# Rinoahu/SwiftOrtho

Hardware: AMD Instinct MI355X
Metric: M query-aa/s scanned all-vs-all (higher is better)
Workload: dtype u8/int16/int32 (5-bit packed residues, packed 16-bit score-only DP, int32 traced DP); 1 GPU; BASELINE config 3: 100000 synthetic proteins x 300 aa self-search, seed 11111011111, aa9, -M 120000000, -c 50000 (2 chunks), -e 1e-5, -v 500; query_aa=30007201, rows=1618760

## Files before the change

### include/sohit.h

```cpp
#ifndef SOHIT_H
#define SOHIT_H

#include <stdint.h>

#ifdef __cplusplus
extern "C" {
#endif

#define SOHIT_ABI_VERSION 3

typedef struct so_ctx so_ctx;

typedef struct so_params {
    const char *seeds;
    const char *alphabet;
    int64_t nc;
    int64_t chunk;
    int64_t step;
    int64_t max_hits;
    int64_t thr;
    double expect;
    double max_miss;
    int32_t filter;
    int32_t profile;
// ... 35 lines not shown
    int64_t bounds_bytes;
    int64_t align_launches;
    double align_ms;
    double index_ms, seed_ms, group_ms, phase2_ms, total_ms;
    int64_t count_launches;
    double count_ms;
    int64_t hits_bucketed;
    int64_t align_wide;
    int64_t cells_wide;
    int64_t seed_passes;
    int64_t ungap_steps;
    int64_t groups_single;
    int64_t groups_chain;
    int64_t bgroup_launches;
    double bgroup_ms;
} so_counters;

so_ctx *so_create(int device, const so_params *params);
void so_destroy(so_ctx *ctx);
const char *so_last_error(const so_ctx *ctx);
int so_abi_version(void);
int so_set_option(so_ctx *ctx, const char *name, const char *value);

int so_load_ref(so_ctx *ctx, const char *fasta_path, int64_t r_lo, int64_t r_hi);
int so_load_ref_mem(so_ctx *ctx, const char *fasta_bytes, int64_t nbytes, int64_t r_lo, int64_t r_hi);
int so_build_index(so_ctx *ctx);
int so_drop_index(so_ctx *ctx);
int so_load_index(so_ctx *ctx, const char *prefix);

int so_load_queries(so_ctx *ctx, const char *fasta_path);
// ... 83 lines not shown
```

### swiftortho_amd/_lib.py

```python
import ctypes as C
import os

HERE = os.path.dirname(os.path.abspath(__file__))
LIBPATH = os.path.join(HERE, "libsohit.so")


class SoParams(C.Structure):
    _fields_ = [("seeds", C.c_char_p), ("alphabet", C.c_char_p), ("nc", C.c_int64), ("chunk", C.c_int64), ("step", C.c_int64),
                ("max_hits", C.c_int64), ("thr", C.c_int64), ("expect", C.c_double), ("max_miss", C.c_double),
                ("filter", C.c_int32), ("profile", C.c_int32)]


class SoHit(C.Structure):
    _fields_ = [("qidx", C.c_int64), ("sidx", C.c_int64), ("identity", C.c_double), ("evalue", C.c_double), ("aln", C.c_int32),
                ("mis", C.c_int32), ("gap", C.c_int32), ("qst", C.c_int32), ("qed", C.c_int32), ("sst", C.c_int32),
                ("sed", C.c_int32), ("bit", C.c_int32), ("qlen", C.c_int32), ("slen", C.c_int32), ("matches", C.c_int32),
                ("ungapped", C.c_int32)]


class SoCounters(C.Structure):
    _fields_ = [(n, C.c_int64) for n in ("n_queries", "query_aa", "ref_seqs", "ref_aa", "n_chunks", "seed_windows", "seed_hits",
                                         "groups", "candidates", "alignments", "cells", "rows", "index_entries")] + \
               [("lookup_launches", C.c_int64), ("lookup_ms", C.c_double), ("lookup_bytes", C.c_int64),
                ("bounds_launches", C.c_int64), ("bounds_ms", C.c_double), ("bounds_bytes", C.c_int64),
                ("align_launches", C.c_int64), ("align_ms", C.c_double),
                ("index_ms", C.c_double), ("seed_ms", C.c_double), ("group_ms", C.c_double), ("phase2_ms", C.c_double),
                ("total_ms", C.c_double), ("count_launches", C.c_int64), ("count_ms", C.c_double),
                ("hits_bucketed", C.c_int64), ("align_wide", C.c_int64), ("cells_wide", C.c_int64), ("seed_passes", C.c_int64),
                ("ungap_steps", C.c_int64), ("groups_single", C.c_int64), ("groups_chain", C.c_int64),
                ("bgroup_launches", C.c_int64), ("bgroup_ms", C.c_double)]

    def as_dict(self):
        return {n: getattr(self, n) for n, _ in self._fields_}


EXPORTS = ["so_abi_version", "so_set_option", "so_create", "so_destroy", "so_last_error", "so_load_ref", "so_load_ref_mem", "so_build_index", "so_drop_index", "so_load_index",
           "so_load_queries", "so_load_queries_mem", "so_num_queries", "so_num_refs", "so_query_len", "so_search_loaded",
           "so_search", "so_free_hits", "so_search_loaded_aln", "so_free_aln", "so_write_sc", "so_format_hit", "so_get_counters", "so_reset_counters", "so_timing_report",
           "so_chunk_threshold", "so_chunk_entries", "so_chunk_download", "so_masked_query", "so_query_candidates", "so_align_pairs", "so_align_pairs_aln", "so_set_profile",
           "so_bucket_count", "so_ref_len", "so_search_device", "so_device_hits_copy", "so_query_work", "so_mcl", "so_mcl_free",
           "so_mcl_last_error", "so_tsv_lines", "so_tsv_scan", "so_tsv_codes", "so_format_pairs", "so_py_repr", "so_fmt_rows",
           "so_search_loaded_cigar", "so_free_cigar", "so_format_cigar", "so_write_sc_cigar", "so_align_pairs_cigar",
           "so_apc", "so_apc_free", "so_apc_last_error"]


# ... 118 lines not shown
```

### swiftortho_amd/build.py

```python
import concurrent.futures
import os
import subprocess
import sys

HERE = os.path.dirname(os.path.abspath(__file__))
CSRC = os.path.join(HERE, "csrc")
OBJ = os.path.join(HERE, "_build")
LIB = os.path.join(HERE, "libsohit.so")
INCLUDE = os.path.join(os.path.dirname(HERE), "include")
HIPCC = os.environ.get("HIPCC", "/opt/rocm/bin/hipcc")
ARCH = "gfx950"

SOURCES = ["k_util.hip", "k_sort.hip", "k_sortseg.hip", "k_prep.hip", "k_index.hip", "k_ixsort.hip", "k_seed.hip", "k_group.hip", "k_ungap1.hip", "k_ungapq.hip", "k_bucket.hip", "k_align.hip", "k_align16.hip", "k_alignl.hip", "k_phase2.hip", "mcl.hip", "apc.hip",
           "tsv.hip", "host_load.hip", "host_index.hip", "host_seed.hip", "host_phase2.hip", "host_search.hip", "host_abi.hip"]
FLAGS = ["-O3", "-std=c++17", "-fPIC", "--offload-arch=" + ARCH, "-ffp-contract=off", "-Wall", "-Wno-unused-function",
         "-Wno-unused-result", "-I", CSRC, "-I", INCLUDE] + os.environ.get("SOHIT_CXXFLAGS", "").split()


def _deps_mtime():
    m = 0.0
    for d in (CSRC, INCLUDE):
        for f in os.listdir(d):
            if f.endswith((".h", ".hpp")):
                m = max(m, os.path.getmtime(os.path.join(d, f)))
    return m


def _compile(src, force):
# ... 33 lines not shown
```

### swiftortho_amd/csrc/host.h

```cpp
#pragma once
#include "common.h"
#include "kernels.h"
#include "seedhash.h"
#include "../../include/sohit.h"

#include <algorithm>
#include <array>
#include <atomic>
#include <chrono>
#include <cmath>
#include <cstring>
#include <functional>
#include <map>
#include <malloc.h>
#include <memory>
#include <mutex>
#include <thread>
#include <unordered_map>
#include <sys/stat.h>

inline double wall() { return std::chrono::duration<double>(std::chrono::steady_clock::now().time_since_epoch()).count(); }

extern double (*volatile p_pow)(double, double);
extern double (*volatile p_log)(double);
// ... 116 lines not shown
    };
    std::vector<std::unique_ptr<RangeTab>> rtabs;
};


#define EMIT_PARTS_MAX 8
enum SmallSlot : int {
    SM_STASH0 = 0, SM_STASH1 = 1,
    SM_SEED_TOTAL = 2,
    SM_ANY_RANK = 3,
    SM_PART_ROW = 4,
    SM_WIDE_ROUND = 12,
    SM_LANE_CTR = 13,
    SM_FLAG = 14,
    SM_WIDE_PART = 16,
    SM_WORDS = 32
};
static_assert(SM_PART_ROW > SM_ANY_RANK && SM_PART_ROW + EMIT_PARTS_MAX <= SM_WIDE_ROUND, "d_small: emission rows");
static_assert(SM_WIDE_PART > SM_FLAG && SM_WIDE_PART + EMIT_PARTS_MAX <= SM_WORDS, "d_small: wide counts per range");

struct so_ctx {
    int device = 0;
    u32 ncu = 256;
    Tune tune;
    hipStream_t st = nullptr;
    std::string seeds, alphabet;
    i64 nc = 0, chunk = 50000, step = 1, v = 500, thr = -1;
    double expect = 1e-3, max_miss = 1e-3;
    bool filter = true, profile = false;
    SeedCfg cfg;
    std::vector<std::array<int, 256>> codes;
    std::string err;
    DevBuf<u8> d_smap, d_hmap;
    DevBuf<signed char> d_b62c;
// ... 163 lines not shown
    DevBuf<u32> cand_q, cand_rec;
    std::vector<u32> chunk_base;
    DevBuf<u32> ccnt;
    DevBuf<unsigned long long> qcells;
    DevBuf<u32> tpos, spcnt, spoff, sidx, spec_trace, sel_a, sel_b;
    DevBuf<u64> gx;
    DevBuf<u32> gL, gR;
    DevBuf<u32> segfirst, st_state, rcnt, tcnt, roff, ridx, ridx2, ntile, roffc, rk_slot, order_tmp;
    DevBuf<u32> cqoff, prior, qtot, qcoff, fin_rec, perm, ntask, toff, sel, nout, ooff;
    DevBuf<AlnTask> tasks;
    DevBuf<AlnRes> ares;
    DevBuf<int> bits, outrec;
    DevBuf<u32> trace;
    DevBuf<u32> tr_units, tr_ofs;
    DevBuf<u32> tl_sorted, al_sorted;
    AlnChain aln;
};

#define QCLASSES 5
static_assert(QCLASSES <= QCLASSES_MAX, "Batch::cls_start");
inline u8 query_class(u32 len) { return len < 512 ? 0 : len < 1024 ? 1 : len < 2048 ? 2 : len < 4096 ? 3 : 4; }

struct StageClock {
    so_ctx* c;
    double t = 0;
    explicit StageClock(so_ctx* c_) : c(c_) {
        if (c->profile) {
            (void)hipStreamSynchronize(c->st);
            t = wall();
        }
// ... 270 lines not shown
```

### swiftortho_amd/csrc/host_phase2.hip

```cpp
#include "host.h"


void aln_decode(const u32* w, int AL, const u8* qp, const u8* sp, char* sq, char* ss) {
    for (int f = 0; f < AL; ++f) {
        const int cc = AL - 1 - f;
        const u32 code = (w[cc >> 4] >> ((cc & 15) << 1)) & 3u;
        sq[f] = code != 2 ? (char)*qp++ : '-';
        ss[f] = code != 3 ? (char)*sp++ : '-';
    }
}

void emit_join(so_ctx* c, HitBuf& out) {
    if (!c->emit.active) return;
    c->emit.th.join();
    c->emit.active = false;
    if (c->emit.err) {
        std::exception_ptr e = c->emit.err;
        c->emit.err = nullptr;
        std::rethrow_exception(e);
    }
    if (c->emit.dropped.load()) {
        const double expect = c->expect;
        if (c->emit.cig) {
            CigarBuf& g = out.cig;
// ... 69 lines not shown
template <class F>
static std::vector<size_t> aln_word_offsets(size_t n, F aln_at, size_t words, const char* who) {
    std::vector<size_t> w(n + 1, 0);
    for (size_t i = 0; i < n; ++i) w[i + 1] = w[i] + (size_t)(std::max(0, (int)aln_at(i)) + 15) / 16;
    if (w[n] != words) throw SoError(std::string(who) + ": column words do not add up");
    return w;
}

struct P2 {
    P2(so_ctx* c, const Batch& b) : sc(c), nq(b.nq) {}
    const double t0 = wall();
    StageClock sc;
    u32 nq, Ntot = 0, NT = 0, nspec = 0, NO = 0;
    AlnSeqs seqs{};
    bool align_sort = false, pk_on = false, pk_mixed = false, lane_on = false, traced_pk = false, aln_on = false, cig_on = false;
    u32 stride = 0, slab = 0, TU = 0;
    size_t var_budget_words = 0, aln_words = 0, cig_ops = 0;
    int parts = 1; u32 qstep = 0;
    std::array<u32, EMIT_PARTS_MAX + 1> part_row{};
    std::vector<u32> h_ooff;
};

static bool gather_candidates(so_ctx* c, Batch& b, P2& p) {
    const int nchunks = (int)c->chunks.size();
    const u32 nq = p.nq;
    const u32 Ntot = p.Ntot = b.chunk_base.empty() ? 0u : b.chunk_base.back();
    b.qtot.ensure((size_t)nq + 4), b.qcoff.ensure((size_t)nq + 4), b.prior.ensure((size_t)nq + 4), b.cqoff.ensure((size_t)nq + 4);
    HIP_CHECK(hipMemsetAsync(b.qtot.p, 0, ((size_t)nq + 4) * sizeof(u32), c->st));
    for (int ci = 0; ci < nchunks; ++ci) launch_add_u32(b.qtot.p, b.ccnt.p + (size_t)ci * nq, nq, c->st);
    c->d_scan_tmp.ensure(scan_u32_temp_elems((size_t)nq + 1) + 8);
// ... 11 lines not shown
        launch_add_u32(b.prior.p, cc, nq, c->st);
    }
    p.sc.lap("phase2.gather");
    if (tune().keep_cands) {
        std::vector<u32> qcoff((size_t)nq + 1), rec(4 * (size_t)Ntot + 4);
        HIP_CHECK(hipMemcpyAsync(qcoff.data(), b.qcoff.p, ((size_t)nq + 1) * sizeof(u32), hipMemcpyDeviceToHost, c->st));
        if (Ntot) HIP_CHECK(hipMemcpyAsync(rec.data(), b.fin_rec.p, 4 * (size_t)Ntot * sizeof(u32), hipMemcpyDeviceToHost, c->st));
        HIP_CHECK(hipStreamSynchronize(c->st));
        for (u32 q = 0; q < nq; ++q) {
            auto& dst = c->last_cands[(size_t)(b.q_lo - c->last_q_lo) + b.qid[q]];
            dst.assign(rec.begin() + 4 * (size_t)qcoff[q], rec.begin() + 4 * (size_t)qcoff[q + 1]);
        }
    }
    return Ntot != 0;
}

static void make_tasks(so_ctx* c, Batch& b, P2& p) {
    const u32 nq = p.nq, Ntot = p.Ntot;
    const u32 vmax = (u32)std::max<i64>(100, std::max<i64>(c->v + 100, (i64)((double)c->v * 1.1)));
    b.perm.ensure((size_t)Ntot + 4), b.ntask.ensure((size_t)nq + 4), b.ntile.ensure((size_t)nq + 4);
    b.toff.ensure((size_t)nq + 4), b.roffc.ensure((size_t)nq + 4);
    HIP_CHECK(hipMemsetAsync(b.ntask.p, 0, ((size_t)nq + 4) * sizeof(u32), c->st));
    HIP_CHECK(hipMemsetAsync(b.ntile.p, 0, ((size_t)nq + 4) * sizeof(u32), c->st));
    if (c->h_qhits_cap < nq) {
        if (c->h_qhits) (void)hipHostFree(c->h_qhits);
        c->h_qhits_cap = (size_t)nq + 1024;
        HIP_CHECK(hipHostMalloc((void**)&c->h_qhits, c->h_qhits_cap * sizeof(unsigned long long), hipHostMallocDefault));
    }
    const u32* qt = reinterpret_cast<const u32*>(c->h_qhits);
    HIP_CHECK(hipMemcpyAsync(c->h_qhits, b.qtot.p, (size_t)nq * sizeof(u32), hipMemcpyDeviceToHost, c->st));
// ... 35 lines not shown
    p.pk_on = tune().align_pk && align_pk_supported(c->st);
    p.pk_mixed = p.pk_on && (int)std::min(maxwin_q, maxwin_s) > align_pk_max_len();
    p.seqs = AlnSeqs{aln_side(b.dev), aln_side(c->ref), c->d_b62c.p};
    p.lane_on = p.pk_on && tune().align_lane && b.maxqlen < LONG_SEQ && c->ref.maxlen < LONG_SEQ;
    p.traced_pk = p.pk_on;
    p.stride = align_trace_stride((int)std::min<u32>(std::max(maxwin_q, maxwin_s), std::min(maxwin_q, maxwin_s) + 16) + 1);
    const long long trace_var_max = tune().trace_var_max;
    const size_t budget_words = trace_var_max >= 0 ? (size_t)trace_var_max : (size_t)1 << 30;
    p.slab = (u32)std::max<size_t>(16, std::min<size_t>(std::max<u32>(NT, 1), budget_words / std::max<u32>(p.stride, 1)));
    p.var_budget_words = trace_var_max >= 0 ? (size_t)trace_var_max : (size_t)1 << 31;
    p.TU = align_trace_unit();
    b.st_state.ensure(5 * (size_t)nq + 8), b.rcnt.ensure((size_t)nq + 4), b.tcnt.ensure((size_t)nq + 4), b.roff.ensure((size_t)nq + 4);
    b.order_tmp.ensure((size_t)nq + 4);
    b.ridx.ensure((size_t)NT + 4);
    HIP_CHECK(hipMemsetAsync(b.st_state.p, 0, (5 * (size_t)nq + 8) * sizeof(u32), c->st));
    p.sc.lap("phase2.mktasks");
}

static void order_by_rows(so_ctx* c, Batch& b, const AlnSeqs& s, const u32* in, u32 n, u32* out, u32* n_wide, unsigned long long* cells) {
    if (!n) return;
    b.tmp64.ensure((size_t)n + 2), b.c_ft2.ensure((size_t)n + 2);
    ensure_sort_tmp(c, sort_pairs_u64_u32_temp_bytes(n, 64));
    launch_task_rows(b.tasks.p, in, n, s, n_wide, cells, b.tmp64.p, c->st);
    sort_pairs_u64_u32(c->d_sort_tmp.p, c->d_sort_tmp.cap, b.tmp64.p, b.c_ft2.p, in, out, n, n_wide ? 14 : 13, c->st);
}

static const u32* round_list(so_ctx* c, Batch& b, const P2& p, const u32* list, u32 n, u32* n_wide) {
    const bool split = n_wide && p.pk_mixed;
    if (n_wide) *n_wide = p.pk_on ? 0u : n;
    if (!split && (!p.align_sort || n < 4096)) return list;
    b.ridx2.ensure((size_t)n + 2);
// ... 13 lines not shown
}

static void align_rounds(so_ctx* c, Batch& b, P2& p) {
    const u32 nq = p.nq, NT = p.NT;
    const AlnSeqs& s = p.seqs;
    u32 aligned_total = 0;
    const bool spec_on = tune().spec >= 0 ? tune().spec != 0 : NT >= (1u << 21);
    const double spec_slack = tune().spec_slack;
    u32 spec_cap = NT;
    if (tune().spec_cap >= 0) spec_cap = (u32)tune().spec_cap;
    if (spec_on) {
        b.tpos.ensure((size_t)NT + 4);
        HIP_CHECK(hipMemsetAsync(b.tpos.p, 0xFF, ((size_t)NT + 4) * sizeof(u32), c->st));
    }
    bool first_round = true;
    for (u32 minr = 8;; minr = minr < 256 ? minr * 2 : minr) {
        u32 NR = 0, RR = 0, NS = 0;
        bool spec_round = spec_on && first_round;
        first_round = false;
        if (spec_round) {
            b.spcnt.ensure((size_t)nq + 4), b.spoff.ensure((size_t)nq + 4), b.sidx.ensure((size_t)NT + 4);
            c->d_small.ensure(SM_WORDS);
            HIP_CHECK(hipMemsetAsync(c->d_small.p + SM_ANY_RANK, 0, sizeof(u32), c->st));
            launch_round_counts_spec(b.ntask.p, b.ntile.p, b.roffc.p, b.rk_slot.p, b.qcoff.p, b.st_state.p, nq, c->max_miss, minr, b.tasks.p, b.toff.p,
                                     b.dev.d_off.p, c->ref.d_off.p, c->d_bittab.p, so_ctx::BITTAB_N, c->ref.N, c->expect * spec_slack, b.rcnt.p, b.tcnt.p, b.spcnt.p,
                                     c->d_small.p + SM_ANY_RANK, c->st);
            stash_u32(c, scan_u32(b.tcnt.p, b.roff.p, (size_t)nq + 1, false, c->d_scan_tmp.p, c->st), SM_STASH0);
            stash_u32(c, scan_u32(b.spcnt.p, b.spoff.p, (size_t)nq + 1, false, c->d_scan_tmp.p, c->st), SM_STASH1);
            u32* v = (u32*)small_host(c);
            HIP_CHECK(hipMemcpyAsync(v, c->d_small.p, (SM_ANY_RANK + 1) * sizeof(u32), hipMemcpyDeviceToHost, c->st));
            HIP_CHECK(hipStreamSynchronize(c->st));
            NR = v[SM_STASH0], NS = v[SM_STASH1], RR = v[SM_ANY_RANK];
            if (NS > spec_cap) spec_round = false;
        }
        if (!spec_round) {
            NS = 0;
            launch_round_counts(b.ntask.p, b.ntile.p, b.roffc.p, b.rk_slot.p, b.qcoff.p, b.st_state.p, nq, c->max_miss, minr, b.rcnt.p,
                                b.tcnt.p, c->st);
            const u32* dNR = scan_u32(b.tcnt.p, b.roff.p, (size_t)nq + 1, false, c->d_scan_tmp.p, c->st);
            stash_u32(c, dNR, SM_STASH0);
            const u32* dRR = scan_u32(b.rcnt.p, b.order_tmp.p, (size_t)nq + 1, false, c->d_scan_tmp.p, c->st);
            d2h_pair(c, dRR, NR, RR);
        }
        if (RR == 0) break;
        if (spec_round) {
            launch_round_idx_spec(b.tcnt.p, b.spcnt.p, b.roff.p, b.spoff.p, b.toff.p, b.ntask.p, b.ntile.p, b.roffc.p, b.rk_slot.p, b.st_state.p, nq,
                                  b.ridx.p, b.sidx.p, c->st);
            if (NS) {
                u32 nw_s = 0;
                const u32* slist = round_list(c, b, p, b.sidx.p, NS, p.traced_pk ? &nw_s : nullptr);
                if (!p.traced_pk) nw_s = NS;
                const size_t tw = trace_offsets(c, b, p, slist, NS);
                ProfTimer pt(c, &c->cnt.align_ms, &c->cnt.align_launches);
                if (tw <= p.var_budget_words) {
                    b.spec_trace.ensure(tw + 64);
                    launch_align_traced(b.tasks.p, slist, NS, s, b.spec_trace.p, p.TU, b.tr_ofs.p, b.ares.p, b.tpos.p, 0u, c->st, nw_s);
                    p.nspec = NS;
                } else {
                    if (tune().debug) fprintf(stderr, "[sohit] kept traces do not fit: %u tasks scored only\n", NS);
                    launch_align(b.tasks.p, slist, NS, s, b.ares.p, c->st);
                }
                pt.stop();
            }
        } else if (NR) {
            launch_round_idx(b.tcnt.p, b.roff.p, b.toff.p, b.ntask.p, b.ntile.p, b.roffc.p, b.rk_slot.p, b.st_state.p, nq, b.ridx.p, c->st);
        }
        if (NR) {
            u32 n_wide = 0;
            const u32* rlist = round_list(c, b, p, b.ridx.p, NR, &n_wide);
            ProfTimer pt(c, &c->cnt.align_ms, &c->cnt.align_launches);
            const bool wide_aside = n_wide && NR > n_wide;
            hipStream_t wst = wide_aside ? c->st_side : c->st;
            if (wide_aside) {
                HIP_CHECK(hipEventRecord(c->ev_ug_go, c->st));
                HIP_CHECK(hipStreamWaitEvent(c->st_side, c->ev_ug_go, 0));
            }
            if (n_wide) launch_align(b.tasks.p, rlist, n_wide, s, b.ares.p, wst);
            if (wide_aside) HIP_CHECK(hipEventRecord(c->ev_ug_done, c->st_side));
            if (NR > n_wide) {
                if (p.lane_on && (long long)(NR - n_wide) >= tune().align_lane_min) {
                    c->d_small.ensure(SM_WORDS);
                    launch_align_lane(b.tasks.p, rlist + n_wide, NR - n_wide, s, b.ares.p, c->d_small.p + SM_LANE_CTR, c->ncu, c->st);
                } else {
                    launch_align_pk(b.tasks.p, rlist + n_wide, NR - n_wide, s, b.ares.p, c->st);
                }
            }
            if (wide_aside) HIP_CHECK(hipStreamWaitEvent(c->st, c->ev_ug_done, 0));
            pt.stop();
            c->cnt.align_wide += n_wide;
        }
        launch_stop_round_w(b.tasks.p, b.ares.p, b.qcoff.p, b.ntask.p, b.ntile.p, b.roffc.p, b.rk_slot.p, b.toff.p, b.rcnt.p, nq,
                            b.dev.d_off.p, c->ref.d_off.p, c->d_bittab.p, so_ctx::BITTAB_N, c->ref.N, c->expect, c->max_miss, c->v, b.sel.p,
                            b.st_state.p, b.bits.p, b.qcells.p, c->st);
        aligned_total += NR + NS;
    }
    launch_sum_u64(b.qcells.p, nq, b.ucount.p + 1, c->st);
    p.sc.lap("phase2.align_rounds");
    c->cnt.alignments += aligned_total;
}

static void select_rows(so_ctx* c, Batch& b, P2& p) {
    const u32 nq = p.nq;
    b.nout.ensure((size_t)nq + 4), b.ooff.ensure((size_t)nq + 4);
    HIP_CHECK(hipMemsetAsync(b.nout.p, 0xFF, (size_t)nq * sizeof(u32), c->st));
    HIP_CHECK(hipMemsetAsync(b.nout.p + nq, 0, 4 * sizeof(u32), c->st));
    launch_final_select(b.toff.p, nq, c->v, b.sel.p, b.st_state.p, b.bits.p, b.nout.p, c->st);
    const u32* dNO = scan_u32(b.nout.p, b.ooff.p, (size_t)nq + 1, false, c->d_scan_tmp.p, c->st);
    const int emit_parts = std::min<int>(EMIT_PARTS_MAX, std::max(1, (p.nspec && (b.permuted || p.pk_mixed)) ? 2 : (int)tune().emit_parts));
    const u32 emit_min_rows = (u32)std::max(1ll, tune().emit_min_rows);
    const u32 qstep = p.qstep = (nq + emit_parts - 1) / emit_parts;
    c->d_small.ensure(SM_WORDS);
    launch_stride_gather(b.ooff.p, qstep, (nq + qstep - 1) / qstep, c->d_small.p + SM_PART_ROW, c->st);
    stash_u32(c, dNO, SM_STASH0);
// ... 488 lines not shown
```

### swiftortho_amd/csrc/host_search.hip

```cpp
#include "host.h"

HitCache g_hit_cache;
BufCache g_cig_ops_cache, g_cig_off_cache;


void search_loaded(so_ctx* c, i64 q_lo, i64 q_hi, HitBuf& out) {
    if (!c->ref_loaded) throw SoError("so_search: no reference loaded");
    if (!c->qry_loaded) throw SoError("so_search: no queries loaded");
    build_index(c);
    struct EmitGuard {
        so_ctx* c;
        ~EmitGuard() {
            if (c->emit.active) {
                c->emit.th.join();
                c->emit.active = false;
                c->emit.err = nullptr;
            }
        }
    } emit_guard{c};
    const double t0 = wall();
    const i64 N = c->qry.N, D = c->ref.N;
    i64 st = std::min<i64>(std::max<i64>(0, q_lo), N);
    i64 ed = std::min<i64>(q_hi < 0 ? D : q_hi, N);
    if (ed < st) ed = st;
// ... 16 lines not shown
    if (tune().batch <= 0) batch_q = std::min<i64>(batch_q, std::max<i64>(1024, (i64)((double)0xE0000000ull / est_cands)));
    std::function<void(i64, i64)> run_batch = [&](i64 b0, i64 b1) {
        const so_counters keep = c->cnt;
        const size_t keep_rows = out.n, keep_dev_rows = c->d_hits_n;
        try {
            if (!c->batch) c->batch = std::make_shared<Batch>();
            Batch& b = *static_cast<Batch*>(c->batch.get());
            b.chunk_base.clear();
            StageClock scp(c);
            prepare_batch(c, b, b0, b1);
            scp.lap("prepare_batch");
            b.ccnt.ensure((size_t)std::max(1, nchunks) * b.nq + 4);
            HIP_CHECK(hipMemsetAsync(b.ccnt.p, 0, ((size_t)std::max(1, nchunks) * b.nq + 4) * sizeof(u32), c->st));
            for (int ci = 0; ci < nchunks; ++ci) seed_stage(c, b, ci);
            phase2(c, b, out);
            unsigned long long uc[3] = {0, 0, 0};
            HIP_CHECK(hipMemcpyAsync(uc, b.ucount.p, sizeof uc, hipMemcpyDeviceToHost, c->st));
            HIP_CHECK(hipStreamSynchronize(c->st));
            c->cnt.cells += (i64)uc[1];
            c->cnt.cells_wide += (i64)uc[2];
            c->cnt.n_queries += b.nq;
            c->cnt.query_aa += b.h_off[b.nq];
            if (tune().keep_masked) {
                if (c->masked.empty()) c->masked_lo = st;
                if (b.h_res.empty() && b.h_off[b.nq]) {
                    b.h_res.resize(b.h_off[b.nq] + 16);
                    HIP_CHECK(hipMemcpy(b.h_res.data(), b.dev.d_res.p, b.h_off[b.nq], hipMemcpyDeviceToHost));
                }
                const size_t m0 = c->masked.size();
                c->masked.resize(m0 + b.nq);
                for (u32 i = 0; i < b.nq; ++i)
                    c->masked[m0 + b.qid[i]].assign((const char*)b.h_res.data() + b.h_off[i], (size_t)(b.h_off[i + 1] - b.h_off[i]));
            }
        } catch (const SoError& e) {
            const bool oom = dynamic_cast<const DevOom*>(&e) != nullptr;
// ... 54 lines not shown
```

### swiftortho_amd/csrc/kernels.h

```cpp
#pragma once
#include "common.h"

struct HashLut;

size_t scan_u32_temp_elems(size_t n);
size_t effscan_temp_elems(size_t n);
const u32* effscan(const u8* mark, const u32* scnt, size_t n, u32* hoff, u32* cidx, u32* temp, hipStream_t st);
const u32* scan_u32(const u32* in, u32* out, size_t n, bool inclusive, u32* temp, hipStream_t st);
void fill_u32(u32* p, size_t n, u32 v, hipStream_t st);

size_t sort_keys_u64_temp_bytes(size_t n, int bits);
void sort_keys_u64(void* temp, size_t temp_bytes, const u64* in, u64* out, size_t n, int begin_bit, int end_bit, hipStream_t st);
void launch_query_segments(const u32* hoff, const u32* qoff, u32 qa, u32 qb, int AS, u32 H, u32* seg, hipStream_t st);
size_t sort_keys_u64_seg_temp_bytes(size_t n, u32 nseg, int begin_bit, int end_bit);
void sort_keys_u64_seg(void* temp, size_t temp_bytes, const u64* in, u64* out, size_t n, u32 nseg, const u32* seg, int begin_bit,
                       int end_bit, hipStream_t st);
void sort_keys_u64_seg2(void* temp, size_t temp_bytes, const u64* in, u64* out, size_t n, u32 nseg, const u32* seg_begin, const u32* seg_end, int begin_bit,
                        int end_bit, hipStream_t st);
void launch_stride_gather(const u32* src, u32 stride, u32 n, u32* dst, hipStream_t st);
size_t sort_pairs_u64_u32_temp_bytes(size_t n, int bits);
void sort_pairs_u64_u32(void* temp, size_t temp_bytes, const u64* kin, u64* kout, const u32* vin, u32* vout, size_t n, int bits,
                        hipStream_t st);

size_t ixsort_plan_elems(u32 NC);
// ... 188 lines not shown
                           const u32* roffc, const u32* rk_slot, const u32* st_state, u32 nq, u32* ridx, u32* sidx, hipStream_t st);
void launch_trace_flags(const u32* sel_idx, u32 n, const u32* tpos, u32* flags, hipStream_t st);
void launch_trace_split(const u32* sel_idx, u32 n, const u32* flags, const u32* fscan, u32* list_b, u32* list_a, hipStream_t st);
u32 aln_unit_words();
void launch_aln_units(const AlnTask* tasks, const u32* sel_idx, u32 n, const AlnSeqs& s, u32* units , hipStream_t st);
void launch_aln_scatter(const u32* sel_idx, u32 n, const u32* rofs, u32* aofs , hipStream_t st);
void launch_aln_words(const u32* sel_idx, u32 n, const AlnRes* res, u32* words , hipStream_t st);
void launch_aln_compact(const u32* sel_idx, u32 n, const u32* aofs, const u32* acode, const u32* cofs , u32* dst, hipStream_t st);
void launch_cigar_count(const u32* sel_idx, u32 n, const u32* aofs, const u32* acode, const AlnRes* res, u32* runs , hipStream_t st);
void launch_cigar_emit(const u32* sel_idx, u32 n, const u32* aofs, const u32* acode, const AlnRes* res, const u32* op_off , u32* ops, hipStream_t st);
void launch_stop_round_w(const AlnTask* tasks, const AlnRes* res, const u32* qcoff, const u32* ntask, const u32* ntile, const u32* roffc,
                         const u32* rk_slot, const u32* toff, const u32* rcnt, u32 nq, const u32* qoff, const u32* roff, const int* bittab,
                         int bittab_n, i64 D, double expect, double max_miss, i64 v, u32* sel, u32* st_state, int* bits,
                         unsigned long long* qcells , hipStream_t st);
void launch_sum_u64(const unsigned long long* x, u32 n, unsigned long long* total, hipStream_t st);
void launch_task_rows(const AlnTask* tasks, const u32* ridx, u32 n, const AlnSeqs& s, u32* n_wide, unsigned long long* cells_wide ,
                      u64* keys, hipStream_t st);
```

### swiftortho_amd/csrc/tune.h

```cpp
#pragma once
#include <cstdlib>

#define SOHIT_TUNE_TABLE(X)                                                                                                                                     \
                                                                                                                              \
    X(B, ug1, "SOHIT_UG1", 1, "bucketed passes: singleton groups to k_ungap1 (0: everything to k_ungap)")                                                     \
    X(B, ug1_chain, "SOHIT_UG1_CHAIN", 1, "... and the groups of two and more hits to k_ungap2 (0: to k_ungap, which then skips the singletons)")              \
    X(B, count_steps, "SOHIT_UG_COUNT", 0, "counting instances of the extension kernels: so_counters.ungap_steps, groups_single, groups_chain")                \
    X(B, ungapq, "SOHIT_UNGAPQ", 1, "sparse passes of queries up to 512 residues: hits alone on their diagonal by k_ungapq, a wave per query (0: every hit through the sorted keys)")     \
    X(B, ug_w32, "SOHIT_UG_W32", 1, "bucketed passes hand k_ungap the buckets' 32-bit words (0: 64-bit keys; no k_ungap1 then)")                               \
                                                                                                             \
    X(B, bucket, "SOHIT_BUCKET", 1, "bucketed diagonal binning (0: every pass on the sorted path)")                                                            \
    X(I, bucket_min, "SOHIT_BUCKET_MIN", 192, "hits per bucket below which a pass takes the sorted path (0: bucketed whenever possible)")                      \
    X(I, bucket_avg, "SOHIT_BUCKET_AVG", 2560, "average bucket size the band-range width is chosen for")                                                       \
    X(I, count_tab, "SOHIT_COUNT_TAB", 1, "bucketed passes: hits per (tile, range) from the range boundaries of the ordered index buckets when a batch brings a chunk two passes and more (0: always the counting pass over the entries; 2: always both, compared -- tests; 3: always)") \
    X(B, bucket_best, "SOHIT_BUCKET_BEST", 1, "best diagonal per subject by the per-bucket reduction (0: sort of the pass records)")                           \
    X(B, bands, "SOHIT_BANDS", 1, "diagonal bands follow the subjects' lengths (0: one band per subject)")                                                     \
    X(B, lk_wide, "SOHIT_LK_WIDE", 0, "8-byte index addends whatever the field widths")                                                                        \
    X(B, qclass, "SOHIT_QCLASS", 1, "queries of a batch in length-class order (0: file order)")                                                                \
    X(B, pass_merge, "SOHIT_PASS_MERGE", 1, "neighbouring length classes that take the sorted path anyway share one pass")                                     \
    X(B, ksc_lazy, "SOHIT_KSC_LAZY", 1, "k-mer orders computed for the queries that reach their frequency cap, when they do (a query below it keeps every window whatever the order; 0: for every query, with the batch)") \
    X(B, bounds_ahead, "SOHIT_BOUNDS_AHEAD", 1, "the next chunk's bucket bounds (k_bounds) on the side stream beside this chunk's seed stage (0: in front of its own)")     \
    X(I, segsort, "SOHIT_SEGSORT", 1, "sorted path: segmented sort of the keys inside each query (0: device-wide sort)")                                        \
    X(I, write_threads, "SOHIT_WRITE_THREADS", 48, "so_write_sc: formatter threads (at most the host's cores)")                                                                          \
                                                                                                                                 \
    X(I, cand_limit, "SOHIT_CAND_LIMIT", 0, "tests: candidate-store size at which a batch is split (0: 2^32 - 16)")                                            \
                                                                                                                                         \
    X(B, align_pk, "SOHIT_ALIGN_PK", 1, "packed 16-bit score-only aligner where the scores fit")                                                               \
    X(B, align_lane, "SOHIT_ALIGN_LANE", 1, "score-only rounds: one lane per alignment pair (k_align_lane) when no sequence reaches 4096 residues (0: k_align_pk)")            \
    X(I, align_lane_min, "SOHIT_ALIGN_LANE_MIN", 1 << 18, "... for rounds of at least this many packed tasks (below: k_align_pk; tests: 0)")                 \
    X(B, align_sort, "SOHIT_ALIGN_SORT", 1, "launch lists ordered by band rows")                                                                               \
    X(I, trace_wave_rows, "SOHIT_TRACE_WAVE_ROWS", 1024, "traceback: bands of this many rows and more are walked by a wave of their own (0: never)")         \
    X(I, trace_wave_max, "SOHIT_TRACE_WAVE_MAX", 32768, "... among the first this many positions of a launch list")                                            \
    X(I, spec, "SOHIT_SPEC", -1, "speculative traces in the first round: 0 off, 1 on, -1 from 2^21 tasks on")                                                  \
    X(D, spec_slack, "SOHIT_SPEC_SLACK", 1e6, "... the guess tests the ungapped score against expect x this (tests: 1e30 = every first-round task traced, 1e-30 = none)")          \
    X(I, spec_cap, "SOHIT_SPEC_CAP", -1, "tests: most speculative traces kept (-1: all)")                                                                      \
    X(I, trace_var_max, "SOHIT_TRACE_VAR_MAX", -1, "tests: trace words a launch list's own-size traces may take, and the fixed-stride slabs' budget (-1: 2^31 / 2^30)") \
    X(I, emit_parts, "SOHIT_EMIT_PARTS", 4, "... and otherwise")                                                                                               \
    X(I, emit_min_rows, "SOHIT_EMIT_MIN_ROWS", 1 << 18, "rows below which the emission is one part")                                                           \
    X(P, test_oom_phase2, "SOHIT_TEST_OOM_PHASE2", 0, "tests: phase 2 of the first batch fails once with an out-of-memory error")                              \
                                                                                                                                 \
    X(I, batch, "SOHIT_BATCH", 0, "queries per device batch (0: 131072, lowered when the candidate estimate asks)")                                            \
    X(I, max_hits, "SOHIT_MAX_HITS", 0, "seed hits per pass (0: 2^30)")                                                                                        \
    X(I, poison, "SOHIT_POISON", -1, "tests: byte every fresh device allocation is filled with (-1: none)")                                                    \
    X(B, hit_cache, "SOHIT_HIT_CACHE", 1, "one released result array is kept for the next search")                                                             \
    X(P, keep_cands, "SOHIT_KEEP_CANDS", 0, "tests: keep every query's candidate list (so_query_candidates)")                                                  \
    X(P, keep_masked, "SOHIT_KEEP_MASKED", 0, "tests: keep the masked queries (so_masked_query)")                                                              \
    X(I, mcl_scratch, "SOHIT_MCL_SCRATCH", -1, "tests: u32 words of expansion / convergence scratch per range of rows (-1: 2^28)")                             \
                                                                                                                                           \
    X(P, exact_threshold, "SOHIT_EXACT_THRESHOLD", 0, "threshold always by the sequential fp64 replay")                                                        \
    X(I, dir_max, "SOHIT_DIR_MAX", -1, "largest -M served by the bitmap + rank directory (-1: 2^31)")                                                          \
// ... 34 lines not shown
```

Baseline: 670.1 M query-aa/s.

## Reuse mirrored pair scores in all-vs-all score-only alignment rounds

In all-vs-all searches, finds for each score-only alignment task its mirrored task (query and subject swapped, same anchor) through a device hash table. Each round it launches only one task of every mirrored pair and copies the max score and cells to the other, avoiding roughly half of the packed DP work. It adds per-batch identity checks, hash insert/probe kernels, per-round mark/filter/copy kernels and a host sync per round. Eligibility is restricted to full-length, non-symmetric-overhang, non-long tasks so the copied score matches what the kernel would compute.

```diff
diff --git a/include/sohit.h b/include/sohit.h
--- a/include/sohit.h
+++ b/include/sohit.h
@@ -73,6 +73,9 @@
     int64_t groups_chain;
     int64_t bgroup_launches;
     double bgroup_ms;
+    int64_t align_reused;
+    int64_t cells_reused;
+    int64_t align_reused_round;
 } so_counters;
 
 so_ctx *so_create(int device, const so_params *params);
diff --git a/swiftortho_amd/_lib.py b/swiftortho_amd/_lib.py
--- a/swiftortho_amd/_lib.py
+++ b/swiftortho_amd/_lib.py
@@ -28,7 +28,8 @@
                 ("total_ms", C.c_double), ("count_launches", C.c_int64), ("count_ms", C.c_double),
                 ("hits_bucketed", C.c_int64), ("align_wide", C.c_int64), ("cells_wide", C.c_int64), ("seed_passes", C.c_int64),
                 ("ungap_steps", C.c_int64), ("groups_single", C.c_int64), ("groups_chain", C.c_int64),
-                ("bgroup_launches", C.c_int64), ("bgroup_ms", C.c_double)]
+                ("bgroup_launches", C.c_int64), ("bgroup_ms", C.c_double),
+                ("align_reused", C.c_int64), ("cells_reused", C.c_int64), ("align_reused_round", C.c_int64)]
 
     def as_dict(self):
         return {n: getattr(self, n) for n, _ in self._fields_}
diff --git a/swiftortho_amd/build.py b/swiftortho_amd/build.py
--- a/swiftortho_amd/build.py
+++ b/swiftortho_amd/build.py
@@ -11,7 +11,7 @@
 HIPCC = os.environ.get("HIPCC", "/opt/rocm/bin/hipcc")
 ARCH = "gfx950"
 
-SOURCES = ["k_util.hip", "k_sort.hip", "k_sortseg.hip", "k_prep.hip", "k_index.hip", "k_ixsort.hip", "k_seed.hip", "k_group.hip", "k_ungap1.hip", "k_ungapq.hip", "k_bucket.hip", "k_align.hip", "k_align16.hip", "k_alignl.hip", "k_phase2.hip", "mcl.hip", "apc.hip",
+SOURCES = ["k_util.hip", "k_sort.hip", "k_sortseg.hip", "k_prep.hip", "k_index.hip", "k_ixsort.hip", "k_seed.hip", "k_group.hip", "k_ungap1.hip", "k_ungapq.hip", "k_bucket.hip", "k_align.hip", "k_align16.hip", "k_alignl.hip", "k_phase2.hip", "k_pair.hip", "mcl.hip", "apc.hip",
            "tsv.hip", "host_load.hip", "host_index.hip", "host_seed.hip", "host_phase2.hip", "host_search.hip", "host_abi.hip"]
 FLAGS = ["-O3", "-std=c++17", "-fPIC", "--offload-arch=" + ARCH, "-ffp-contract=off", "-Wall", "-Wno-unused-function",
          "-Wno-unused-result", "-I", CSRC, "-I", INCLUDE] + os.environ.get("SOHIT_CXXFLAGS", "").split()
diff --git a/swiftortho_amd/csrc/host.h b/swiftortho_amd/csrc/host.h
--- a/swiftortho_amd/csrc/host.h
+++ b/swiftortho_amd/csrc/host.h
@@ -154,10 +154,11 @@
     SM_LANE_CTR = 13,
     SM_FLAG = 14,
     SM_WIDE_PART = 16,
+    SM_PAIR = 24,
     SM_WORDS = 32
 };
 static_assert(SM_PART_ROW > SM_ANY_RANK && SM_PART_ROW + EMIT_PARTS_MAX <= SM_WIDE_ROUND, "d_small: emission rows");
-static_assert(SM_WIDE_PART > SM_FLAG && SM_WIDE_PART + EMIT_PARTS_MAX <= SM_WORDS, "d_small: wide counts per range");
+static_assert(SM_WIDE_PART > SM_FLAG && SM_WIDE_PART + EMIT_PARTS_MAX <= SM_PAIR && SM_PAIR + 4 <= SM_WORDS, "d_small: wide counts per range, mirrored tasks");
 
 struct so_ctx {
     int device = 0;
@@ -351,6 +352,9 @@
     DevBuf<u32> trace;
     DevBuf<u32> tr_units, tr_ofs;
     DevBuf<u32> tl_sorted, al_sorted;
+    DevBuf<u8> pr_same;
+    DevBuf<u32> pr_partner, pr_state, pr_launch, pr_copy;
+    DevBuf<u64> pr_tab;
     AlnChain aln;
 };
 
diff --git a/swiftortho_amd/csrc/host_phase2.hip b/swiftortho_amd/csrc/host_phase2.hip
--- a/swiftortho_amd/csrc/host_phase2.hip
+++ b/swiftortho_amd/csrc/host_phase2.hip
@@ -107,6 +107,7 @@
     u32 nq, Ntot = 0, NT = 0, nspec = 0, NO = 0;
     AlnSeqs seqs{};
     bool align_sort = false, pk_on = false, pk_mixed = false, lane_on = false, traced_pk = false, aln_on = false, cig_on = false;
+    bool pair_on = false;
     u32 stride = 0, slab = 0, TU = 0;
     size_t var_budget_words = 0, aln_words = 0, cig_ops = 0;
     int parts = 1; u32 qstep = 0;
@@ -148,6 +149,8 @@
     }
     return Ntot != 0;
 }
+
+static bool pair_lookup(so_ctx* c, Batch& b, const P2& p);
 
 static void make_tasks(so_ctx* c, Batch& b, P2& p) {
     const u32 nq = p.nq, Ntot = p.Ntot;
@@ -213,7 +216,28 @@
     b.order_tmp.ensure((size_t)nq + 4);
     b.ridx.ensure((size_t)NT + 4);
     HIP_CHECK(hipMemsetAsync(b.st_state.p, 0, (5 * (size_t)nq + 8) * sizeof(u32), c->st));
+    p.pair_on = p.pk_on && b.maxqlen < LONG_SEQ && c->ref.maxlen < LONG_SEQ && b.q_lo < c->ref.N &&
+                (tune().pair_reuse >= 0 ? tune().pair_reuse != 0 : NT >= (1u << 18)) && pair_lookup(c, b, p);
     p.sc.lap("phase2.mktasks");
+}
+
+static bool pair_lookup(so_ctx* c, Batch& b, const P2& p) {
+    const u32 nq = p.nq, NT = p.NT;
+    c->d_small.ensure(SM_WORDS);
+    b.pr_same.ensure((size_t)nq + 4);
+    HIP_CHECK(hipMemsetAsync(c->d_small.p + SM_PAIR + 3, 0, sizeof(u32), c->st));
+    const u32* qid = b.permuted ? b.d_qid.p : nullptr;
+    launch_pair_same(p.seqs, nq, (u32)b.q_lo, qid, (u32)c->ref.N, b.pr_same.p, c->d_small.p + SM_PAIR + 3, c->st);
+    const u32 n_same = d2h_u32(c, c->d_small.p + SM_PAIR + 3);
+    if (tune().debug) fprintf(stderr, "[sohit] pair reuse: %u of %u queries are their own reference sequences\n", n_same, nq);
+    if (n_same < 2) return false;
+    const size_t entries = pair_table_entries(NT);
+    b.pr_tab.ensure(entries), b.pr_partner.ensure((size_t)NT + 4), b.pr_state.ensure((size_t)NT + 4);
+    b.pr_launch.ensure((size_t)NT + 4), b.pr_copy.ensure((size_t)NT + 4);
+    HIP_CHECK(hipMemsetAsync(b.pr_tab.p, 0xFF, entries * sizeof(u64), c->st));
+    HIP_CHECK(hipMemsetAsync(b.pr_state.p, 0, ((size_t)NT + 4) * sizeof(u32), c->st));
+    launch_pair_lookup(b.tasks.p, NT, p.seqs, b.pr_same.p, (u32)b.q_lo, nq, qid, b.pr_tab.p, b.pr_partner.p, c->st);
+    return true;
 }
 
 static void order_by_rows(so_ctx* c, Batch& b, const AlnSeqs& s, const u32* in, u32 n, u32* out, u32* n_wide, unsigned long long* cells) {
@@ -257,6 +281,8 @@
         HIP_CHECK(hipMemsetAsync(b.tpos.p, 0xFF, ((size_t)NT + 4) * sizeof(u32), c->st));
     }
     bool first_round = true;
+    u32 pair_tag = 0;
+    u32 pair_scored = 0, pair_reused = 0, pair_round = 0;
     for (u32 minr = 8;; minr = minr < 256 ? minr * 2 : minr) {
         u32 NR = 0, RR = 0, NS = 0;
         bool spec_round = spec_on && first_round;
@@ -286,9 +312,30 @@
             d2h_pair(c, dRR, NR, RR);
         }
         if (RR == 0) break;
-        if (spec_round) {
+        if (spec_round)
             launch_round_idx_spec(b.tcnt.p, b.spcnt.p, b.roff.p, b.spoff.p, b.toff.p, b.ntask.p, b.ntile.p, b.roffc.p, b.rk_slot.p, b.st_state.p, nq,
                                   b.ridx.p, b.sidx.p, c->st);
+        else if (NR)
+            launch_round_idx(b.tcnt.p, b.roff.p, b.toff.p, b.ntask.p, b.ntile.p, b.roffc.p, b.rk_slot.p, b.st_state.p, nq, b.ridx.p, c->st);
+        u32 NL = NR;
+        const u32* score_list = b.ridx.p;
+        if (p.pair_on && NR + NS) {
+            ++pair_tag;
+            launch_pair_mark(b.ridx.p, NR, b.sidx.p, NS, pair_tag, b.pr_state.p, c->st);
+            if (NR) {
+                HIP_CHECK(hipMemsetAsync(c->d_small.p + SM_PAIR, 0, 3 * sizeof(u32), c->st));
+                launch_pair_filter(b.ridx.p, NR, pair_tag, b.pr_partner.p, b.pr_state.p, b.pr_launch.p, b.pr_copy.p, c->d_small.p + SM_PAIR, c->st);
+                u32* v = (u32*)small_host(c);
+                HIP_CHECK(hipMemcpyAsync(v, c->d_small.p + SM_PAIR, 3 * sizeof(u32), hipMemcpyDeviceToHost, c->st));
+                HIP_CHECK(hipStreamSynchronize(c->st));
+                NL = v[0];
+                if (NL > NR || v[1] != NR - NL) throw SoError("phase 2: the split of a round's mirrored tasks does not add up");
+                score_list = b.pr_launch.p;
+                pair_scored += NR, pair_reused += NR - NL, pair_round += v[2];
+                if (tune().debug) fprintf(stderr, "[sohit] pair round %u: %u score-only tasks, %u launched, %u copied (%u from this round)\n", pair_tag, NR, NL, NR - NL, v[2]);
+            }
+        }
+        if (spec_round) {
             if (NS) {
                 u32 nw_s = 0;
                 const u32* slist = round_list(c, b, p, b.sidx.p, NS, p.traced_pk ? &nw_s : nullptr);
@@ -305,14 +352,12 @@
                 }
                 pt.stop();
             }
-        } else if (NR) {
-            launch_round_idx(b.tcnt.p, b.roff.p, b.toff.p, b.ntask.p, b.ntile.p, b.roffc.p, b.rk_slot.p, b.st_state.p, nq, b.ridx.p, c->st);
-        }
-        if (NR) {
+        }
+        if (NL) {
             u32 n_wide = 0;
-            const u32* rlist = round_list(c, b, p, b.ridx.p, NR, &n_wide);
+            const u32* rlist = round_list(c, b, p, score_list, NL, &n_wide);
             ProfTimer pt(c, &c->cnt.align_ms, &c->cnt.align_launches);
-            const bool wide_aside = n_wide && NR > n_wide;
+            const bool wide_aside = n_wide && NL > n_wide;
             hipStream_t wst = wide_aside ? c->st_side : c->st;
             if (wide_aside) {
                 HIP_CHECK(hipEventRecord(c->ev_ug_go, c->st));
@@ -320,18 +365,19 @@
             }
             if (n_wide) launch_align(b.tasks.p, rlist, n_wide, s, b.ares.p, wst);
             if (wide_aside) HIP_CHECK(hipEventRecord(c->ev_ug_done, c->st_side));
-            if (NR > n_wide) {
-                if (p.lane_on && (long long)(NR - n_wide) >= tune().align_lane_min) {
+            if (NL > n_wide) {
+                if (p.lane_on && (long long)(NL - n_wide) >= tune().align_lane_min) {
                     c->d_small.ensure(SM_WORDS);
-                    launch_align_lane(b.tasks.p, rlist + n_wide, NR - n_wide, s, b.ares.p, c->d_small.p + SM_LANE_CTR, c->ncu, c->st);
+                    launch_align_lane(b.tasks.p, rlist + n_wide, NL - n_wide, s, b.ares.p, c->d_small.p + SM_LANE_CTR, c->ncu, c->st);
                 } else {
-                    launch_align_pk(b.tasks.p, rlist + n_wide, NR - n_wide, s, b.ares.p, c->st);
+                    launch_align_pk(b.tasks.p, rlist + n_wide, NL - n_wide, s, b.ares.p, c->st);
                 }
             }
             if (wide_aside) HIP_CHECK(hipStreamWaitEvent(c->st, c->ev_ug_done, 0));
             pt.stop();
             c->cnt.align_wide += n_wide;
         }
+        if (p.pair_on && NR) launch_pair_copy(b.pr_launch.p, NL, b.pr_copy.p, NR - NL, b.pr_partner.p, b.ares.p, b.pr_state.p, b.ucount.p + 3, c->st);
         launch_stop_round_w(b.tasks.p, b.ares.p, b.qcoff.p, b.ntask.p, b.ntile.p, b.roffc.p, b.rk_slot.p, b.toff.p, b.rcnt.p, nq,
                             b.dev.d_off.p, c->ref.d_off.p, c->d_bittab.p, so_ctx::BITTAB_N, c->ref.N, c->expect, c->max_miss, c->v, b.sel.p,
                             b.st_state.p, b.bits.p, b.qcells.p, c->st);
@@ -340,6 +386,10 @@
     launch_sum_u64(b.qcells.p, nq, b.ucount.p + 1, c->st);
     p.sc.lap("phase2.align_rounds");
     c->cnt.alignments += aligned_total;
+    c->cnt.align_reused += pair_reused, c->cnt.align_reused_round += pair_round;
+    if (p.pair_on && tune().debug)
+        fprintf(stderr, "[sohit] pair reuse: %u score-only tasks in %u rounds, %u took their mirrored task's result (%u from the same round)\n", pair_scored,
+                pair_tag, pair_reused, pair_round);
 }
 
 static void select_rows(so_ctx* c, Batch& b, P2& p) {
diff --git a/swiftortho_amd/csrc/host_search.hip b/swiftortho_amd/csrc/host_search.hip
--- a/swiftortho_amd/csrc/host_search.hip
+++ b/swiftortho_amd/csrc/host_search.hip
@@ -54,11 +54,12 @@
             HIP_CHECK(hipMemsetAsync(b.ccnt.p, 0, ((size_t)std::max(1, nchunks) * b.nq + 4) * sizeof(u32), c->st));
             for (int ci = 0; ci < nchunks; ++ci) seed_stage(c, b, ci);
             phase2(c, b, out);
-            unsigned long long uc[3] = {0, 0, 0};
+            unsigned long long uc[4] = {0, 0, 0, 0};
             HIP_CHECK(hipMemcpyAsync(uc, b.ucount.p, sizeof uc, hipMemcpyDeviceToHost, c->st));
             HIP_CHECK(hipStreamSynchronize(c->st));
             c->cnt.cells += (i64)uc[1];
             c->cnt.cells_wide += (i64)uc[2];
+            c->cnt.cells_reused += (i64)uc[3];
             c->cnt.n_queries += b.nq;
             c->cnt.query_aa += b.h_off[b.nq];
             if (tune().keep_masked) {
diff --git a/swiftortho_amd/csrc/k_pair.hip b/swiftortho_amd/csrc/k_pair.hip
--- /dev/null
+++ b/swiftortho_amd/csrc/k_pair.hip
@@ -0,0 +1,182 @@
+#include "common.h"
+#include "kernels.h"
+
+#define PAIR_NONE 0xFFFFFFFFu
+#define PAIR_PENDING 0xFFFFFFFEu
+#define PAIR_DONE 0xFFFFFFFFu
+#define PAIR_EMPTY (~0ull)
+
+__global__ __launch_bounds__(64) void k_pair_same(const u8* __restrict__ q_pcls, const u8* __restrict__ q_pcls4, const u32* __restrict__ qoff,
+                                                  const u8* __restrict__ r_pcls, const u8* __restrict__ r_pcls4, const u32* __restrict__ roff,
+                                                  u32 q_lo, const u32* __restrict__ qid, u32 nref, u8* __restrict__ same, u32* __restrict__ n_same) {
+    const u32 s = blockIdx.x, lane = threadIdx.x;
+    const u32 rel = qid ? qid[s] : s;
+    const u64 g = (u64)q_lo + rel;
+    bool eq = g < nref;
+    if (eq) {
+        const u32 a = qoff[s], len = qoff[s + 1] - a, ra = roff[g];
+        eq = len == roff[g + 1] - ra;
+        if (eq) {
+            const size_t qo = (size_t)a + (size_t)PCLS_PAD * s, ro = (size_t)ra + (size_t)PCLS_PAD * g;
+            for (u32 i = lane; i < len + PCLS_PAD; i += 64) eq = eq && q_pcls[qo + i] == r_pcls[ro + i] && q_pcls4[qo + i] == r_pcls4[ro + i];
+        }
+    }
+    eq = __all(eq);
+    if (lane == 0) {
+        same[rel] = eq ? 1 : 0;
+        if (eq) atomicAdd(n_same, 1u);
+    }
+}
+
+__device__ __forceinline__ u64 pair_hash(u32 a, u32 b, u32 qi, u32 qj) {
+    u64 x = ((u64)a << 32 | b) ^ (((u64)qi << 32 | qj) * 0x9E3779B97F4A7C15ull);
+    x ^= x >> 32, x *= 0xD6E8FEB86659FD93ull;
+    x ^= x >> 32, x *= 0xD6E8FEB86659FD93ull;
+    return x ^ (x >> 32);
+}
+
+struct PairArgs {
+    const AlnTask* tasks;
+    u32 ntasks;
+    const u32 *qoff, *roff, *qbound, *rbound;
+    int pk_len;
+    u32 pk_score;
+    const u8* same;
+    u32 q_lo, nq;
+    const u32* qid;
+    u64* tab;
+    u32 mask;
+};
+
+__device__ __forceinline__ u32 pair_ordinal(const PairArgs& a, u32 q) { return a.q_lo + (a.qid ? a.qid[q] : q); }
+
+__device__ __forceinline__ bool pair_eligible(const PairArgs& a, const AlnTask& tk) {
+    const u32 srel = tk.subj - a.q_lo;
+    if (tk.subj < a.q_lo || srel >= a.nq) return false;
+    if (!a.same[a.qid ? a.qid[tk.q] : tk.q] || !a.same[srel]) return false;
+    const u32 lq = a.qoff[tk.q + 1] - a.qoff[tk.q], ls = a.roff[tk.subj + 1] - a.roff[tk.subj];
+    if (lq >= LONG_SEQ || ls >= LONG_SEQ || tk.qe != lq || tk.se != ls) return false;
+    const u32 la = lq - min(tk.qi, lq), lb = ls - min(tk.qj, ls);
+    if (la == lb) return false;
+    return !((int)min(la, lb) > a.pk_len && min(a.qbound[tk.q], a.rbound[tk.subj]) > a.pk_score);
+}
+
+__global__ __launch_bounds__(256) void k_pair_insert(const PairArgs a, u32* __restrict__ partner) {
+    const u32 t = blockIdx.x * 256u + threadIdx.x;
+    if (t >= a.ntasks) return;
+    const AlnTask tk = a.tasks[t];
+    const bool el = pair_eligible(a, tk);
+    partner[t] = el ? PAIR_PENDING : PAIR_NONE;
+    if (!el) return;
+    const u64 h = pair_hash(pair_ordinal(a, tk.q), tk.subj, tk.qi, tk.qj);
+    const u64 e = (h & 0xFFFFFFFF00000000ull) | t;
+    for (u32 i = (u32)h & a.mask;; i = (i + 1u) & a.mask)
+        if (atomicCAS((unsigned long long*)(a.tab + i), (unsigned long long)PAIR_EMPTY, (unsigned long long)e) == PAIR_EMPTY) break;
+}
+
+__global__ __launch_bounds__(256) void k_pair_probe(const PairArgs a, u32* __restrict__ partner) {
+    const u32 t = blockIdx.x * 256u + threadIdx.x;
+    if (t >= a.ntasks || partner[t] != PAIR_PENDING) return;
+    const uint4 tk = *reinterpret_cast<const uint4*>(a.tasks + t);
+    const u32 gq = pair_ordinal(a, tk.x);
+    const u64 h = pair_hash(tk.y, gq, tk.w, tk.z);
+    u32 found = PAIR_NONE;
+    for (u32 i = (u32)h & a.mask;; i = (i + 1u) & a.mask) {
+        const u64 e = a.tab[i];
+        if (e == PAIR_EMPTY) break;
+        if ((e >> 32) != (h >> 32)) continue;
+        const u32 p = (u32)e;
+        const uint4 pk = *reinterpret_cast<const uint4*>(a.tasks + p);
+        if (pk.y == gq && pk.z == tk.w && pk.w == tk.z && pair_ordinal(a, pk.x) == tk.y) {
+            found = p;
+            break;
+        }
+    }
+    partner[t] = found;
+}
+
+__global__ __launch_bounds__(256) void k_pair_mark(const u32* __restrict__ ridx, u32 nr, const u32* __restrict__ sidx, u32 ns, u32 tag,
+                                                   u32* __restrict__ state) {
+    const u32 i = blockIdx.x * 256u + threadIdx.x;
+    if (i < nr) state[ridx[i]] = tag;
+    else if (i < nr + ns) state[sidx[i - nr]] = PAIR_DONE;
+}
+
+__global__ __launch_bounds__(256) void k_pair_filter(const u32* __restrict__ ridx, u32 nr, u32 tag, const u32* __restrict__ partner,
+                                                     const u32* __restrict__ state, u32* __restrict__ launch, u32* __restrict__ copy,
+                                                     u32* __restrict__ cnt) {
+    const u32 i = blockIdx.x * 256u + threadIdx.x, lane = threadIdx.x & 63u;
+    u32 t = 0, kind = 0;
+    const bool live = i < nr;
+    if (live) {
+        t = ridx[i];
+        const u32 p = partner[t];
+        if (p != PAIR_NONE) {
+            const u32 sp = state[p];
+            if (sp == PAIR_DONE) kind = 1;
+            else if (sp == tag && p < t) kind = 2;
+            if (kind && partner[p] != t) kind = 0;
+        }
+    }
+    const unsigned long long ml = __ballot(live && !kind), mc = __ballot(live && kind), m2 = __ballot(kind == 2);
+    u32 bl = 0, bc = 0;
+    if (lane == 0) {
+        if (ml) bl = atomicAdd(cnt, (u32)__popcll(ml));
+        if (mc) bc = atomicAdd(cnt + 1, (u32)__popcll(mc));
+        if (m2) atomicAdd(cnt + 2, (u32)__popcll(m2));
+    }
+    bl = __shfl(bl, 0), bc = __shfl(bc, 0);
+    const unsigned long long below = (1ull << lane) - 1ull;
+    if (live && !kind) launch[bl + (u32)__popcll(ml & below)] = t;
+    else if (live) copy[bc + (u32)__popcll(mc & below)] = t;
+}
+
+__global__ __launch_bounds__(256) void k_pair_copy(const u32* __restrict__ launch, u32 nl, const u32* __restrict__ copy, u32 nc,
+                                                   const u32* __restrict__ partner, AlnRes* __restrict__ res, u32* __restrict__ state,
+                                                   unsigned long long* __restrict__ cells_reused) {
+    const u32 i = blockIdx.x * 256u + threadIdx.x;
+    unsigned long long cells = 0;
+    if (i < nl) {
+        state[launch[i]] = PAIR_DONE;
+    } else if (i < nl + nc) {
+        const u32 t = copy[i - nl], p = partner[t];
+        const int ms = res[p].maxscore, nc_ = res[p].cells;
+        res[t].maxscore = ms, res[t].cells = nc_;
+        state[t] = PAIR_DONE;
+        cells = (unsigned long long)(u32)nc_;
+    }
+    if (__ballot(cells != 0)) {
+#pragma unroll
+        for (int o = 32; o > 0; o >>= 1) cells += __shfl_xor(cells, o);
+        if ((threadIdx.x & 63) == 0) atomicAdd(cells_reused, cells);
+    }
+}
+
+void launch_pair_same(const AlnSeqs& s, u32 nq, u32 q_lo, const u32* qid, u32 nref, u8* same, u32* n_same, hipStream_t st) {
+    if (!nq) return;
+    hipLaunchKernelGGL(k_pair_same, dim3(nq), dim3(64), 0, st, s.q.pcls, s.q.pcls4, s.q.off, s.r.pcls, s.r.pcls4, s.r.off, q_lo, qid, nref, same, n_same);
+}
+
+size_t pair_table_entries(u32 ntasks) { return (size_t)1 << ceil_log2(2ull * std::max<u32>(ntasks, 32u)); }
+
+void launch_pair_lookup(const AlnTask* tasks, u32 ntasks, const AlnSeqs& s, const u8* same, u32 q_lo, u32 nq, const u32* qid, u64* tab ,
+                        u32* partner, hipStream_t st) {
+    if (!ntasks) return;
+    const PairArgs a{tasks, ntasks, s.q.off, s.r.off, s.q.bound, s.r.bound, align_pk_max_len(), align_pk_max_score(), same, q_lo, nq, qid, tab,
+                     (u32)(pair_table_entries(ntasks) - 1)};
+    hipLaunchKernelGGL(k_pair_insert, dim3((ntasks + 255) / 256), dim3(256), 0, st, a, partner);
+    hipLaunchKernelGGL(k_pair_probe, dim3((ntasks + 255) / 256), dim3(256), 0, st, a, partner);
+}
+
+void launch_pair_mark(const u32* ridx, u32 nr, const u32* sidx, u32 ns, u32 tag, u32* state, hipStream_t st) {
+    if (nr + ns) hipLaunchKernelGGL(k_pair_mark, dim3((nr + ns + 255) / 256), dim3(256), 0, st, ridx, nr, sidx, ns, tag, state);
+}
+
+void launch_pair_filter(const u32* ridx, u32 nr, u32 tag, const u32* partner, const u32* state, u32* launch, u32* copy, u32* cnt, hipStream_t st) {
+    if (nr) hipLaunchKernelGGL(k_pair_filter, dim3((nr + 255) / 256), dim3(256), 0, st, ridx, nr, tag, partner, state, launch, copy, cnt);
+}
+
+void launch_pair_copy(const u32* launch, u32 nl, const u32* copy, u32 nc, const u32* partner, AlnRes* res, u32* state, unsigned long long* cells_reused,
+                      hipStream_t st) {
+    if (nl + nc) hipLaunchKernelGGL(k_pair_copy, dim3((nl + nc + 255) / 256), dim3(256), 0, st, launch, nl, copy, nc, partner, res, state, cells_reused);
+}
diff --git a/swiftortho_amd/csrc/kernels.h b/swiftortho_amd/csrc/kernels.h
--- a/swiftortho_amd/csrc/kernels.h
+++ b/swiftortho_amd/csrc/kernels.h
@@ -226,5 +226,13 @@
                          int bittab_n, i64 D, double expect, double max_miss, i64 v, u32* sel, u32* st_state, int* bits,
                          unsigned long long* qcells , hipStream_t st);
 void launch_sum_u64(const unsigned long long* x, u32 n, unsigned long long* total, hipStream_t st);
+void launch_pair_same(const AlnSeqs& s, u32 nq, u32 q_lo, const u32* qid , u32 nref, u8* same, u32* n_same, hipStream_t st);
+size_t pair_table_entries(u32 ntasks);
+void launch_pair_lookup(const AlnTask* tasks, u32 ntasks, const AlnSeqs& s, const u8* same, u32 q_lo, u32 nq, const u32* qid, u64* tab ,
+                        u32* partner, hipStream_t st);
+void launch_pair_mark(const u32* ridx, u32 nr, const u32* sidx, u32 ns, u32 tag, u32* state, hipStream_t st);
+void launch_pair_filter(const u32* ridx, u32 nr, u32 tag, const u32* partner, const u32* state, u32* launch, u32* copy, u32* cnt, hipStream_t st);
+void launch_pair_copy(const u32* launch, u32 nl, const u32* copy, u32 nc, const u32* partner, AlnRes* res, u32* state, unsigned long long* cells_reused,
+                      hipStream_t st);
 void launch_task_rows(const AlnTask* tasks, const u32* ridx, u32 n, const AlnSeqs& s, u32* n_wide, unsigned long long* cells_wide ,
                       u64* keys, hipStream_t st);
diff --git a/swiftortho_amd/csrc/tune.h b/swiftortho_amd/csrc/tune.h
--- a/swiftortho_amd/csrc/tune.h
+++ b/swiftortho_amd/csrc/tune.h
@@ -34,6 +34,7 @@
     X(I, spec, "SOHIT_SPEC", -1, "speculative traces in the first round: 0 off, 1 on, -1 from 2^21 tasks on")                                                  \
     X(D, spec_slack, "SOHIT_SPEC_SLACK", 1e6, "... the guess tests the ungapped score against expect x this (tests: 1e30 = every first-round task traced, 1e-30 = none)")          \
     X(I, spec_cap, "SOHIT_SPEC_CAP", -1, "tests: most speculative traces kept (-1: all)")                                                                      \
+    X(I, pair_reuse, "SOHIT_PAIR_REUSE", -1, "all-vs-all: a score-only task takes the score of its mirrored task (subject and query exchanged) of the same batch: 0 off, 1 on, -1 from 2^18 tasks on") \
     X(I, trace_var_max, "SOHIT_TRACE_VAR_MAX", -1, "tests: trace words a launch list's own-size traces may take, and the fixed-stride slabs' budget (-1: 2^31 / 2^30)") \
     X(I, emit_parts, "SOHIT_EMIT_PARTS", 4, "... and otherwise")                                                                                               \
     X(I, emit_min_rows, "SOHIT_EMIT_MIN_ROWS", 1 << 18, "rows below which the emission is one part")                                                           \
```

Measured after the change: 633.5 M query-aa/s. 5.5% lower.
